# YuejiangDong/MAL

Hardware: AMD Instinct MI355X
Metric: train images/sec at B=12 192x640 KITTI-shaped (MAL loss path: passes A+B+C fwd+bwd) (higher is better)
Workload: dtype f32

## Files before the change

include/mal_hip.h:

```cpp
#ifndef MAL_HIP_H
#define MAL_HIP_H

#include <stddef.h>
#include <stdint.h>

#ifdef __cplusplus
extern "C" {
#endif

#define MAL_VERSION 100
#define MAL_MAX_FRAMES 2
#define MAL_MAX_CAND 4
#define MAL_MAX_INSTANCES 64
#define MAL_MATCH_MAX 128
#define MAL_INSTANCES_MAX_QK 16384
#define MAL_INSTANCES_MAX_K1 1025
#define MAL_INSTANCES_MAX_N 65535
#define MAL_MSDA_MAX_L 8
#define MAL_MSDA_MAX_P 8
#define MAL_MSDA_MAX_LP 32
#define MAL_MSDA_MAX_D 64

enum {
  MAL_OK = 0,
// ... 115 lines not shown

int mal_pose_fwd(const float* const* axisangle, const float* const* translation, const int* invert,
                 int B, int F, float* const* T, void* stream);
int mal_pose_bwd(const float* const* axisangle, const float* const* translation, const int* invert,
                 const float* const* g_T, int B, int F, float* const* g_axisangle ,
                 float* const* g_translation , void* stream);

enum {
  MAL_STEP_NO_ENS = 1,
  MAL_STEP_AUG_MASK = 2,
  MAL_STEP_TEMPORAL = 8,
  MAL_STEP_NOISE_PHILOX = 4,
  MAL_STEP_TEXEL_INPUTS = 64,
  MAL_STEP_DUAL_DISTIL = 32,
  MAL_STEP_SYN_SPARSE = 16,
  MAL_STEP_MAIN_TEMPORAL = 128,
  MAL_STEP_SYN_S_SPARSE = 256,
  MAL_STEP_NO_MOTION_MASK = 1024,
  MAL_STEP_NO_AUG = 2048,
  MAL_STEP_ENSEMBLE = 4096,
  MAL_STEP_NO_SSIM = 512
};
typedef struct mal_step_args {
  int B, H, W;
  float min_depth, max_depth;
  int flags;
  float w_main, w_distil;
  const float *color0, *color_m1, *color_p1;
  const float *K, *inv_K;
  const float *disp_teacher, *disp_student;
// ... 319 lines not shown
```

mal_amd/_lib.py:

```python
from __future__ import annotations

import ctypes as C
import os

import torch

_HERE = os.path.dirname(os.path.abspath(__file__))
LIB_PATH = os.environ.get("MAL_HIP_LIB") or os.path.join(_HERE, "lib", "libmal_hip.so")

c_fp = C.c_void_p
c_pp = C.c_void_p
i32, f32, sz, vp = C.c_int, C.c_float, C.c_size_t, C.c_void_p

SIGNATURES = {
    "mal_version": (i32, []),
    "mal_strerror": (C.c_char_p, [i32]),
    "mal_device_check": (i32, []),
    "mal_workspace_bytes": (sz, [i32, i32, i32]),
    "mal_disp_to_depth": (i32, [c_fp, sz, f32, f32, c_fp, c_fp, vp]),
    "mal_disp_to_depth_bwd": (i32, [c_fp, c_fp, c_fp, sz, f32, f32, c_fp, vp]),
    "mal_backproject": (i32, [c_fp, c_fp, i32, i32, i32, c_fp, vp]),
    "mal_backproject_bwd": (i32, [c_fp, c_fp, i32, i32, i32, c_fp, vp]),
    "mal_project3d": (i32, [c_fp, c_fp, c_fp, i32, i32, i32, f32, i32, c_fp, c_fp, vp]),
    "mal_project3d_bwd": (i32, [c_fp, c_fp, c_fp, c_fp, c_fp, i32, i32, i32, f32, i32, c_fp, c_fp, vp, sz, vp]),
# ... 185 lines not shown


class MsdaArgs(C.Structure):
    _fields_ = ([(n, vp) for n in ("value", "spatial_shapes", "level_start_index", "sampling_locations", "attention_weights",
                                   "reference_points")] +
                [(n, i32) for n in ("N", "S", "M", "D", "L", "P", "Lq", "ref_dim")] + [("out", vp), ("stream", vp)])


DR_MAX_ITERS = 4
MATCH_MAX,MATCH_U8, MATCH_F32 = 128, 0, 1
DR_NO_AUTOMASK, DR_NO_MOTION_MASK, DR_NOISE_PHILOX, DR_AVG, DR_NO_SSIM, DR_POSE_UPDATE = 1, 2, 4, 8, 16, 32
DR_POSE_NOISE_KEY = 0x706f73655f757064
MS_MAX_SCALES = 4
STEP_NO_ENS, STEP_AUG_MASK, STEP_NOISE_PHILOX, STEP_TEMPORAL, STEP_SYN_SPARSE, STEP_DUAL_DISTIL, STEP_TEXEL_INPUTS = 1, 2, 4, 8, 16, 32, 64
STEP_MAIN_TEMPORAL, STEP_SYN_S_SPARSE, STEP_NO_SSIM, STEP_NO_MOTION_MASK, STEP_NO_AUG, STEP_ENSEMBLE = 128, 256, 512, 1024, 2048, 4096
DEC_WIN, DEC_DISTIL, DEC_SMOOTH_X, DEC_SMOOTH_Y, DEC_TAP0, DEC_TAP1, DEC_L1, DEC_PLANES = 0, 1, 2, 3, 4, 5, 6, 7

F_AUTOMASK, F_GRAD, F_POSE_GRAD, F_NO_SSIM, F_AVG, F_EPILOGUE, F_DUAL_DISTIL, F_SRC_PACKED, F_TGT_PACKED = 1, 2, 4, 8, 16, 32, 64, 128, 256

_lib = None


class MalError(RuntimeError):
    pass


def load():
    global _lib
    if _lib is not None:
        return _lib
# ... 35 lines not shown
```

mal_amd/config.py:

```python
noise_source = "cpu"
noise_seed = 0x4d414c5eed
consistency_target = True
```

mal_amd/csrc/mal_march.h:

```cpp
#pragma once
#include "mal_common.h"
#include "mal_device.h"
#include "mal_pose.h"

namespace mal {

struct MarchParams {
  const float* disp; const float* disp2; const float* K; const float* invK;
  const float* T[2]; const float* src[2];
  const float* target; const float* ident; const float* noise; const float* ext_mask; const float* sample_scale;
  const float* mono_depth; const float* mono_reproj; const float* ens_reproj;
  const float* mono_disp; const float* lowest_cost; float* cmask_out;
  float merge_cons, merge_distil;
  const float* ens_disp; float* g_ens;
  int dual_distil;
  int avg, no_ssim;
  float* cam; int cam_ready;
  int sample_scale_is_mask;
  int B, H, W; float min_disp, range, eps; int convention;
  float* min_reproj; float* g_reproj; float* g_cons; float* g_distil; float* cons_target; float* depth_out;
  double* block_sums; float* block_gP;
  float* bnd;
  int strips, segs, rows, ntasks, per_xcd;
  int packed;
  int flip_odd;
  int debug;
  float* color_out[2]; unsigned char* argmin_out;
  float* min_reproj2; unsigned char* argmin_out2; float* weight_out;
  int color_out_stride;
  float* color_out2[2];
  const float* forced_w; const unsigned char* forced_arg; const float* g_color[2];
  const unsigned char* region;
  const float* fin_gn; const float* fin_coefs; const double* fin_stats; const float* fin_g_total; float* fin_out;
  unsigned* dbg;
  int framed; float* g_reproj2; float* bnd2;
};
constexpr int kDecPlanes = MAL_DEC_PLANES;

constexpr int kCamFloats = 40;

MAL_DEV void cam_fill(const float* K, const float* T0, const float* T1, const float* invK, float* cam, int b, int lane) {
  float mine = 0.f;
  if (lane < 24) {
    const int f = lane & 1, e = lane >> 1, i = e >> 2, j = e & 3;
    const float* Kb = K + b * 16;
    const float* T = (f ? T1 : T0) + b * 16;
    float acc = Kb[i * 4 + 0] * T[0 * 4 + j];
    acc = fma_(Kb[i * 4 + 1], T[1 * 4 + j], acc);
    acc = fma_(Kb[i * 4 + 2], T[2 * 4 + j], acc);
    mine = fma_(Kb[i * 4 + 3], T[3 * 4 + j], acc);
// ... 2 lines not shown
    mine = invK[b * 16 + (e / 3) * 4 + (e % 3)];
  }
  if (lane < kCamFloats) cam[b * kCamFloats + lane] = mine;
}

MarchParams march_params(int B, int H, int W, float min_depth, float max_depth, float eps, int convention);
int march_launch(MarchParams& p, int flags, hipStream_t st);
bool march_pair_qualifies(int B, int H, int W);
int march_pair_launch(MarchParams* ens, MarchParams& stu, int order, hipStream_t st);
void march_geometry(int B, int H, int W, int flags, int* strips, int* segs, int* rows);
inline int march_tasks_per_sample(int B, int H, int W, int flags) {
  int strips = 0, segs = 0;
  march_geometry(B, H, W, flags, &strips, &segs, nullptr);
  return strips * segs;
}
void step_geom_record(const void* ws, int B, int H, int W);
int step_geom_check(const void* ws, int B, int H, int W);
inline size_t march_bnd_floats(int B, int H, int W) { return (size_t)B * ((size_t)H / 8 + 1) * 2 * (size_t)W; }
MAL_DEV float march_boundary_term(const float* bnd, int b, int y, int x, int H, int W, int rows, int segs) {
  const int sq = y / rows, within = y - sq * rows;
  const int last = min(rows, H - sq * rows) - 1;
  float v = 0.f;
  if (within == 0 && sq > 0) v = bnd[((size_t)(b * segs + sq) * 2 + 0) * W + x];
  else if (within == last && sq < segs - 1) v = bnd[((size_t)(b * segs + sq) * 2 + 1) * W + x];
  return v;
}
MAL_DEV const float* march_boundary_row(const float* bnd, int b, int y, int H, int W, int rows, int segs) {
  const int sq = y / rows, within = y - sq * rows;
  const int last = min(rows, H - sq * rows) - 1;
  if (within == 0 && sq > 0) return bnd + ((size_t)(b * segs + sq) * 2 + 0) * W;
// ... 3 lines not shown
int pack_identity_tasks_per_sample(int H, int W);
struct StepPoses { PoseParams pose; const float* K; const float* invK; float* cam; unsigned* ticket; };
struct TieNoise { int on; unsigned long long seed, step; const unsigned long long* counter; float* noise_out ; };
struct SmoothParams { int n; const float* disp[2]; float* gn[2]; double* partials; unsigned* dec[2]; };
constexpr int kDrSlotsMax = 5;
struct DrExtra {
  const float* K; const float* invK; const float* T[kDrSlotsMax][2]; float* cam[kDrSlotsMax]; float* noise[kDrSlotsMax];
  unsigned long long seed, step; const unsigned long long* counter;
  int slots, pu_slot, noise_blocks, B, H, W; unsigned* ticket;
};
struct FusedMoreArgs {
  const float* target; const float* cand0; const float* cand1; int idx0; const float* ident; const float* noise;
  const float* prev_min; const uint8_t* prev_arg; float* min_reproj; uint8_t* argmin; float* weight_out; double* block_sums;
  float* g_cand0; float* g_cand1; const uint8_t* region; float* g_region0; float* g_region1; const float* orig0; const float* orig1;
  size_t orig_stride; int weight_given;
};
int photo_march_fused_more(const FusedMoreArgs& a, int B, int H, int W, int* per_sample_out, hipStream_t st,
                           unsigned* order = nullptr, unsigned* order_count = nullptr);
int photo_march_fused_more_n(int n, const FusedMoreArgs* a, int B, int H, int W, int* per_sample_out, hipStream_t st);
struct SmoothMapArgs { const float* disp; const float* img; int H, W; float* gn; double* partial; };
int smooth_march_sweep_batch(int n, const SmoothMapArgs* maps, int B, hipStream_t st, int* per_sample);
int smooth_march_batch_tasks(int H, int W);
hipStream_t side_begin(hipStream_t st);
int side_end(hipStream_t st);
int side_wait(hipStream_t st, bool always);
int tiebreak_noise_launch(unsigned long long seed, unsigned long long step, const unsigned long long* counter, unsigned mult,
                          int n, int B, int H, int W, float* const* out, hipStream_t st);
struct UpMaps { const float* src[2 * MAL_MS_MAX_SCALES]; float* dst[2 * MAL_MS_MAX_SCALES]; int h[2 * MAL_MS_MAX_SCALES], w[2 * MAL_MS_MAX_SCALES]; };
struct MsExtra {
  unsigned long long seed, step; const unsigned long long* counter; unsigned mult; int n_noise; float* noise[MAL_MS_MAX_SCALES];
  UpMaps up; int n_up;
// ... 154 lines not shown
```

mal_amd/csrc/mal_march.hip:

```cpp
#include "mal_march.h"
#include <atomic>
#include "mal_device.h"
#include "mal_pairs.h"
#include <mutex>
#include <unordered_map>

namespace mal {

#ifdef MAL_STAGE_MARKS
#define MAL_MARK(n) do { __builtin_amdgcn_sched_barrier(0); asm volatile("; MAL_STAGE " #n); __builtin_amdgcn_sched_barrier(0); } while (0)
#else
#define MAL_MARK(n) do { } while (0)
#endif

typedef __attribute__((address_space(4))) const float cfloat;

MAL_DEV void load_cam(const cfloat* cam, f2 (&P)[12], float (&ik)[9]) {
  asm volatile("" : "+s"(cam));
#pragma unroll
  for (int e = 0; e < 12; ++e) P[e] = (f2){cam[2 * e], cam[2 * e + 1]};
#pragma unroll
  for (int e = 0; e < 9; ++e) ik[e] = cam[24 + e];
}

// ... 373 lines not shown
  };
  auto maps_of = [&](CParams& pp) {
    Maps m;
    m.ident = AUTOMASK ? pp.ident : nullptr; m.noise = (AUTOMASK && !NO_NOISE) ? pp.noise : nullptr;
    m.ext_mask = EXT_NO ? nullptr : pp.ext_mask; m.lowest_cost = COST_NO ? nullptr : pp.lowest_cost;
    m.mono_disp = (COST_NO && !EPI) ? nullptr : pp.mono_disp;
    m.mono_depth = EPI ? pp.mono_depth : nullptr; m.mono_reproj = EPI ? pp.mono_reproj : nullptr;
    m.ens_reproj = EPI ? pp.ens_reproj : nullptr; m.target = pp.target; m.packed = LEAN ? 3 : pp.packed;
    m.forced_w = TEMPORAL ? pp.forced_w : nullptr; m.forced_arg = TEMPORAL ? pp.forced_arg : nullptr;
    m.gcol[0] = TEMPORAL ? pp.g_color[0] : nullptr; m.gcol[1] = TEMPORAL ? pp.g_color[1] : nullptr;
    m.fin_gn = TEMPORAL ? pp.fin_gn : nullptr;
    m.ens_disp = EPI ? pp.ens_disp : nullptr;
    return m;
  };
  auto row_of = [&](int rr) { return min(max(reflect1(rr, H), 0), H - 1); };
  auto request = [&](const Maps& pp, int rr, Ahead& a) {
    const bool packed_t = (pp.packed & 2) != 0;
    const unsigned pix = (unsigned)(prow(row_of(rr)) * W + gxr);
    const unsigned od = moff(row_of(rr));
    a.disp = ldf(disp_b, od);
    a.disp2 = 0.f;
    if (!NO_DISP2) {
      const float v = ldf(disp2_b ? disp2_b : disp_b, od);
      a.disp2 = disp2_b ? v : 0.f;
    }
    load_rgb(pp.target, packed_t, b, HW, pix, a.y);
    const unsigned oc = moff(min(max(rr - 1, 0), H - 1));
    auto opt = [&](const float* m, unsigned off, float absent) {
      const float v = ldf(m ? m : disp_b, off);
      return m ? v : absent;
    };
    a.ident = 0.f; a.noise = 0.f;
    if (AUTOMASK && !TEMPORAL) { a.ident = ldf(pp.ident, oc); if (!NO_NOISE) a.noise = opt(pp.noise, oc, 0.f); }
    if (TEMPORAL) {
      a.ident = ldf(pp.forced_w, oc);
      a.noise = (float)*(pp.forced_arg + (oc >> 2));
      const unsigned og = moff(min(max(rr - 2, 0), H - 1)) + 2u * (unsigned)b * (unsigned)HW * 4u;
#pragma unroll
      for (int ch = 0; ch < 3; ++ch) {
        const unsigned o = og + (unsigned)ch * (unsigned)HW * 4u;
#pragma unroll
        for (int f = 0; f < 2; ++f) a.gc[f * 3 + ch] = ldf(pp.gcol[f], o);
      }
    }
    a.ext = 1.f; a.mono = 0.f; a.cost = 1.f;
    if (EXT_YES) a.ext = ldf(pp.ext_mask, oc);
    else if (!EXT_NO) a.ext = opt(pp.ext_mask, oc, 1.f);
    if (COST_YES) {
      a.mono = ldf(pp.mono_disp, oc); a.cost = ldf(pp.lowest_cost, oc);
    } else if (!COST_NO) {
      a.mono = opt(pp.lowest_cost ? pp.mono_disp : nullptr, oc, 0.f);
      a.cost = opt(pp.lowest_cost, oc, 1.f);
    }
    const unsigned oq = GRAD ? moff(min(max(rr - 2, 0), H - 1)) : oc;
    a.e_mono = 0.f; a.e_mr = 0.f; a.e_er = 0.f; a.e_ensd = 0.f;
    if (EPI) {
      a.e_mono = ldf(MONO_YES ? pp.mono_disp : (pp.mono_disp ? pp.mono_disp : pp.mono_depth), oq);
// ... 969 lines not shown
}

int march_launch(MarchParams& p, int flags, hipStream_t st) {
  const bool grad = flags & MAL_F_GRAD, automask = flags & MAL_F_AUTOMASK, pose = flags & MAL_F_POSE_GRAD,
             epi = flags & MAL_F_EPILOGUE;
  march_decompose(p, flags);
  p.debug = g_debug;
  p.flip_odd = g_march_flip;
  p.packed = ((flags & MAL_F_SRC_PACKED) ? 1 : 0) | ((flags & MAL_F_TGT_PACKED) ? 2 : 0);
  dim3 grid(p.per_xcd * 8), block(64);
  if (!p.cam) return MAL_EINVAL;
  if ((long long)p.H * p.W >= (1ll << 24)) return MAL_ESHAPE;
  if (p.color_out[0] && (long long)p.B * (p.color_out_stride ? (long long)p.color_out_stride : 3ll * p.H * p.W) * 4 >= (1ll << 32))
    return MAL_ESHAPE;
  if (p.forced_w && (long long)p.B * 3 * p.H * p.W * 4 >= (1ll << 32)) return MAL_ESHAPE;
  if (!p.cam_ready) {
    hipLaunchKernelGGL(cam_setup_kernel, dim3(p.B), dim3(64), 0, st, p.K, p.T[0], p.T[1], p.invK, p.cam);
    p.cam_ready = 1;
  }
  const bool named = grad && pose && automask && !epi;
  hipEvent_t ev0 = named ? g_prof_start.exchange(nullptr) : nullptr, ev1 = named ? g_prof_stop.exchange(nullptr) : nullptr;
  if (ev0) (void)hipEventRecord(ev0, st);
  if ((p.avg || p.no_ssim) && (!grad || p.forced_w || p.color_out[0])) return MAL_EINVAL;
  const bool lean0 = g_march_lean && p.packed == 3 && !p.depth_out && p.debug == 0 && !p.dbg && !p.avg && !p.no_ssim &&
                     (long long)p.H * p.W * (kTexel * 4) < (1ll << 24);
  const bool no_maps = !p.ext_mask && !p.lowest_cost && !p.sample_scale;
  const bool conv_a = p.convention == 0, conv_b = p.convention == 1;
#ifdef MAL_CONV_FIXED
  const bool conv_teacher = conv_a;
#else
// ... 204 lines not shown
    if (m.h[k] < 1 || m.w[k] < 1 || m.h[k] > H || m.w[k] > W) return MAL_ESHAPE;
  }
  const MarchParams mp = march_params(B, H, W, min_depth, max_depth, 1e-7f, 0);
  WarpScalesParams p;
  p.m = m; p.src[0] = src[0]; p.src[1] = src[1]; p.cam = cam;
  p.B = B; p.H = H; p.W = W; p.stride = stride > 0 ? stride : 3 * H * W;
  p.min_disp = mp.min_disp; p.range = mp.range;
  const dim3 grid((W + 63) / 64, (H + 3) / 4, B * m.n), block(64, 4);
  if ((long long)H * W * (kTexel * 4) < (1ll << 24)) hipLaunchKernelGGL(warp_scales_kernel<true>, grid, block, 0, st, p);
  else hipLaunchKernelGGL(warp_scales_kernel<false>, grid, block, 0, st, p);
  return launch_status();
}

struct StepGeom {
  int rows_grad, rows_fwd, pack_rows, halo1;
  bool operator==(const StepGeom& o) const {
    return rows_grad == o.rows_grad && rows_fwd == o.rows_fwd && pack_rows == o.pack_rows && halo1 == o.halo1;
  }
};
static StepGeom step_geom_now(int B, int H, int W) {
  StepGeom g = {};
  march_geometry(B, H, W, MAL_F_GRAD, nullptr, nullptr, &g.rows_grad);
  march_geometry(B, H, W, 0, nullptr, nullptr, &g.rows_fwd);
  g.pack_rows = g_pack_rows;
  g.halo1 = g_march_halo1;
  return g;
}
static std::mutex g_geom_mutex;
static std::unordered_map<const void*, StepGeom> g_geom;

void step_geom_record(const void* ws, int B, int H, int W) {
  const StepGeom g = step_geom_now(B, H, W);
  std::lock_guard<std::mutex> lock(g_geom_mutex);
  if (g_geom.size() >= 4096 && !g_geom.count(ws)) g_geom.clear();
  g_geom[ws] = g;
}

int step_geom_check(const void* ws, int B, int H, int W) {
  const StepGeom g = step_geom_now(B, H, W);
  std::lock_guard<std::mutex> lock(g_geom_mutex);
// ... 166 lines not shown
```

mal_amd/csrc/mal_photo_march.hip:

```cpp
#include "mal_common.h"
#include "mal_device.h"
#include "mal_march.h"
#include "mal_pairs.h"

namespace mal {

struct PhotoMarchParams {
  const float* target; const float* cand[2];
  int target_texels;
  int weight_given;
  int idx[2];
  const float* ident; const float* noise; const float* ext_mask;
  const float* prev_min; const uint8_t* prev_arg;
  int last, automask;
  float* min_reproj; uint8_t* argmin; float* weight_out; double* block_sums;
  const uint8_t* argmin_in; const float* weight_in; const float* scale; const double* sums;
  float* g_cand[2];
  int B, H, W, strips, segs, rows, ntasks, per_xcd;
  const uint8_t* region;
  float* g_region[2];
  unsigned* order; unsigned* order_count;
  const float* orig[2]; size_t orig_stride;
};

struct Px9 { float t[3], a[3], c[3]; };

MAL_DEV void request9(const PhotoMarchParams& p, const float* tb, const float* ab, const float* cb, int HW, int row,
                      int gxr, Px9& q) {
  const unsigned bo = (unsigned)(row * p.W + gxr) * 4u;
  if (p.target_texels) {
    const texel_t t = ldt(tb, bo * (unsigned)kTexel);
    q.t[0] = t.x; q.t[1] = t.y; q.t[2] = t.z;
#pragma unroll
    for (int ch = 0; ch < 3; ++ch) { q.a[ch] = ldf(ab + (size_t)ch * HW, bo); q.c[ch] = ldf(cb + (size_t)ch * HW, bo); }
    return;
  }
#pragma unroll
// ... 140 lines not shown
  for (int i = 0; i < 9; ++i) { hsA[i] = bc(0.f); hsB[i] = bc(0.f); hcA[i] = bc(0.f); hcB[i] = bc(0.f); }
#pragma unroll
  for (int i = 0; i < 2; ++i) { hyA[i] = bc(0.f); hyB[i] = bc(0.f); hzA[i] = 0.f; hzB[i] = 0.f; }
  f2 x1[3] = {bc(0.f), bc(0.f), bc(0.f)}, x2[3] = {bc(0.f), bc(0.f), bc(0.f)}, y1rg = bc(0.f), y2rg = bc(0.f);
  float y1b = 0.f, y2b = 0.f;
  float w1 = 0.f;
  int win1 = 255;
  float acc_rw = 0.f, acc_w = 0.f;
  auto row_of = [&](int rr) { return min(max(reflect1(rr, H), 0), H - 1); };
  const uint8_t* rgn0 = (FUSED && p.region) ? p.region + map_b : nullptr;
  if (FUSED && rgn0) {
    unsigned any = 0u;
#pragma unroll 8
    for (int rr = max(y_lo - 2, 0); rr <= min(y_hi + 1, H - 1); ++rr) any |= rgn0[rr * W + gxr];
    if (!__any((any & 1u) && in_x)) {
      if (out_x)
        for (int c = y_lo; c < y_hi; ++c) {
          const unsigned o0 = (unsigned)(c * W + gxr) * 4u + img_b, o1 = o0 + hw4, o2 = o1 + hw4;
          stf(p.g_cand[0], o0, 0.f); stf(p.g_cand[0], o1, 0.f); stf(p.g_cand[0], o2, 0.f);
          if (p.g_cand[1]) { stf(p.g_cand[1], o0, 0.f); stf(p.g_cand[1], o1, 0.f); stf(p.g_cand[1], o2, 0.f); }
        }
      if (lane == 0) { p.block_sums[(size_t)task * 2] = 0.0; p.block_sums[(size_t)task * 2 + 1] = 0.0; }
      return;
    }
  }
  float nfA = 0.f, nfB = 0.f;
  const int r_first = max(y_lo - HALO, -1), r_last = y_hi - 1 + HALO;
  Px9 nxt;
  auto request9o = [&](CPhoto& P, int row, Px9& q) {
    const unsigned bo = (unsigned)(row * W + gxr) * 4u;
    const unsigned o0 = bo + img_b, o1 = o0 + hw4, o2 = o1 + hw4;
    if (FUSED) {
      const texel_t t = ldt(P.target, bo * (unsigned)kTexel + (unsigned)b * (unsigned)HW * (unsigned)(kTexel * 4));
      q.t[0] = t.x; q.t[1] = t.y; q.t[2] = t.z;
    } else {
      q.t[0] = ldf(P.target, o0); q.t[1] = ldf(P.target, o1); q.t[2] = ldf(P.target, o2);
    }
    q.a[0] = ldf(P.cand[0], o0); q.a[1] = ldf(P.cand[0], o1); q.a[2] = ldf(P.cand[0], o2);
    q.c[0] = ldf(P.cand[1], o0); q.c[1] = ldf(P.cand[1], o1); q.c[2] = ldf(P.cand[1], o2);
  };
// ... 423 lines not shown
    PhotoMarchParams p = {};
    p.target = target; p.B = B; p.H = H; p.W = W;
    const bool has2 = 2 * pr + 1 < n_cand;
    int i0 = 2 * pr, i1 = has2 ? 2 * pr + 1 : -1;
    if (!g_cand[i0] && i1 >= 0 && g_cand[i1]) { const int t = i0; i0 = i1; i1 = t; }
    if (!g_cand[i0]) continue;
    p.cand[0] = cand[i0]; p.idx[0] = i0; p.g_cand[0] = g_cand[i0];
    p.cand[1] = i1 >= 0 ? cand[i1] : cand[i0]; p.idx[1] = i1; p.g_cand[1] = i1 >= 0 ? g_cand[i1] : nullptr;
    p.argmin_in = argmin; p.weight_in = weight; p.scale = scale; p.sums = sums;
    decompose(p, 60, 2);
    hipLaunchKernelGGL(photo_march_bwd_kernel<false>, dim3(p.per_xcd * 8), dim3(64), 0, st, p);
  }
  return launch_status();
}

static int fused_more_params(PhotoMarchParams& p, const FusedMoreArgs& x, int B, int H, int W) {
  if (x.prev_min == x.min_reproj || x.prev_arg == x.argmin) return MAL_EINVAL;
  if (x.weight_given && x.noise) return MAL_EINVAL;
  if ((x.orig0 == nullptr) != (x.orig1 == nullptr) || (x.orig0 && !x.region)) return MAL_EINVAL;
  if ((long long)B * 3 * H * W * 4 >= (1ll << 32)) return MAL_ESHAPE;
  const size_t orig_stride = x.orig_stride ? x.orig_stride : (size_t)3 * H * W;
  if (x.orig0 && (long long)B * (long long)orig_stride * 4 >= (1ll << 32)) return MAL_ESHAPE;
  p = PhotoMarchParams{};
  p.target = x.target; p.target_texels = 1;
  p.weight_given = x.weight_given; p.B = B; p.H = H; p.W = W;
  p.cand[0] = x.cand0; p.cand[1] = x.cand1; p.idx[0] = x.idx0; p.idx[1] = x.idx0 + 1;
  p.prev_min = x.prev_min; p.prev_arg = x.prev_arg; p.ident = x.ident; p.noise = x.noise;
  p.min_reproj = x.min_reproj; p.argmin = x.argmin; p.weight_out = x.weight_out; p.block_sums = x.block_sums;
  p.g_cand[0] = x.g_cand0; p.g_cand[1] = x.g_cand1; p.region = x.region;
  p.orig[0] = x.orig0; p.orig[1] = x.orig1; p.orig_stride = orig_stride;
  if (x.region && x.g_region0 && x.g_region1) { p.g_region[0] = x.g_region0; p.g_region[1] = x.g_region1; }
  if (x.region && g_syn_rows >= 2 && g_syn_rows < 8) decompose(p, 60, 8, g_syn_rows);
  else decompose(p, 60, 2);
  return MAL_OK;
}
int photo_march_fused_more(const FusedMoreArgs& a, int B, int H, int W, int* per_sample_out, hipStream_t st, unsigned* order,
                           unsigned* order_count) {
  PhotoMarchParams p = {};
  int rc = fused_more_params(p, a, B, H, W);
  if (rc) return rc;
  *per_sample_out = p.strips * p.segs;
  unsigned grid = (unsigned)p.per_xcd * 8u;
#ifdef MAL_EXPERIMENTS
  if (a.region && order && order_count && g_syn_queue) {
    p.order = order; p.order_count = order_count;
    grid = (unsigned)p.ntasks;
    hipLaunchKernelGGL(photo_march_classify_kernel, dim3(grid), dim3(64), 0, st, p);
  }
#else
// ... 21 lines not shown
```

mal_amd/csrc/mal_step.hip:

```cpp
#include "mal_march.h"
#include "mal_device.h"
#include "mal_pose.h"
#include "mal_pairs.h"
#include "mal_tail.h"
#include <mutex>

namespace mal {

constexpr int kLossSlots = 16;
constexpr int kEpiBlocks = 64;

opt_t g_march_halo1{1};
opt_t g_step_overlap{1};
opt_t g_temporal_spec{0};
opt_t g_side_priority{0};
opt_t g_student_overlap{2};
opt_t g_side_order{0};
opt_t g_tail_overlap{1};
opt_t g_sweeps_batched{1};

struct StepWs {
  float* packed[3];
  float* T[2]; float* gT[2]; float* gTs[2];
  float* ident; float* mono_reproj; float* ens_reproj;
  float* G_r_t; float* G_r_s; float* G_c; float* gn_t; float* gn_s;
  float* G_e;
  float* multi_reproj;
  double* bs_d;
  double* bs_t; double* bs_s; double* bs_e; float* bgP;
  float* bgP_e;
  double* bs_p;
  unsigned char* arg_t; float* w_t; double* bs_ph;
  float* rp_warp; unsigned char* arg_warp;
  unsigned char* arg_s; float* w_s; double* bs_sh; float* rp_warp_s; unsigned char* arg_warp_s;
  double* ps;
  unsigned* ticket;
  unsigned* order;
  double* sm_stats;
  float* coefs;
  float* cam;
  float* bnd_t; float* bnd_s;
  size_t bytes;
};

static StepWs carve_step(void* base, int B, int H, int W) {
  StepWs w;
  char* p = (char*)base;
// ... 16 lines not shown
  w.rp_warp = (float*)take(map);
  w.arg_warp = (unsigned char*)take((size_t)B * HW);
  w.arg_s = (unsigned char*)take((size_t)B * HW);
  w.w_s = (float*)take(map);
  w.bs_sh = (double*)take(nb * 4 * 2 * 8);
  w.rp_warp_s = (float*)take(map);
  w.arg_warp_s = (unsigned char*)take((size_t)B * HW);
  w.ps = (double*)take((size_t)2 * B * 8 * 8);
  w.ticket = (unsigned*)take(16);
  w.order = (unsigned*)take(nb * 4 * sizeof(unsigned));
  w.sm_stats = (double*)take((size_t)4 * B * 8);
  w.coefs = (float*)take(16 * 4);
  w.cam = (float*)take((size_t)B * 40 * 4);
  w.bnd_t = (float*)take(march_bnd_floats(B, H, W) * 4);
  w.bnd_s = (float*)take(march_bnd_floats(B, H, W) * 4);
  w.bytes = o;
  return w;
}

struct EpiParams {
  const float *disp_s, *disp_t, *mono_reproj, *ens_reproj, *multi_reproj, *ext_mask, *lowest_cost, *sample_scale, *ens_disp;
  int scale_is_mask, dual;
  int skip_dead;
  float min_disp, range, merge_cons, merge_distil;
  float *G_c, *G_e; double* partials; unsigned* dbg; int B, HW;
};
MAL_DEV void step_epilogue_block(const EpiParams& p, int bid) {
  __shared__ double s_red[2][4];
  const int b = bid / kEpiBlocks, blk = bid - b * kEpiBlocks, tid = threadIdx.x;
  const int per = (p.HW + kEpiBlocks - 1) / kEpiBlocks, lo = blk * per, hi = min(lo + per, p.HW);
// ... 643 lines not shown
      m.out[k][0] = student ? sc->warp_s_m1[s] : sc->warp_m1[s];
      m.out[k][1] = student ? sc->warp_s_p1[s] : sc->warp_p1[s];
      m.out2[k][0] = student ? sc->warp2_s_m1[s] : sc->warp2_m1[s];
      m.out2[k][1] = student ? sc->warp2_s_p1[s] : sc->warp2_p1[s];
      if (!m.disp[k] || !m.out[k][0] || !m.out[k][1] || (m.out2[k][0] == nullptr) != (m.out2[k][1] == nullptr)) return MAL_EINVAL;
    }
  }
  rc = step_check(a);
  if (rc) return rc;
  const StepWs w = step_ws(a);
  const float* src[2] = {w.packed[1], w.packed[2]};
  return warp_scales_launch(m, src, w.cam, a->B, a->H, a->W, a->min_depth, a->max_depth, a->warp_sample_stride,
                            (hipStream_t)a->stream);
}

static FusedMoreArgs teacher_sweep(const mal_step_args* a, const StepWs& w, float* mono_reproj) {
  const bool sparse = (a->flags & MAL_STEP_SYN_SPARSE) != 0;
  FusedMoreArgs x = {};
  x.target = w.packed[0]; x.cand0 = a->syn_m1; x.cand1 = a->syn_p1; x.idx0 = 2; x.ident = w.ident; x.noise = a->noise;
  x.prev_min = w.rp_warp; x.prev_arg = w.arg_warp; x.min_reproj = mono_reproj; x.argmin = w.arg_t; x.weight_out = w.w_t;
  x.block_sums = w.bs_ph; x.g_cand0 = a->g_syn_m1; x.g_cand1 = a->g_syn_p1; x.region = a->syn_region;
  x.g_region0 = a->g_syn_region_m1; x.g_region1 = a->g_syn_region_p1;
  x.orig0 = sparse ? a->warp_m1 : nullptr; x.orig1 = sparse ? a->warp_p1 : nullptr; x.orig_stride = (size_t)a->warp_sample_stride;
  return x;
}
static FusedMoreArgs student_sweep(const mal_step_args* a, const StepWs& w) {
  const bool sparse = (a->flags & MAL_STEP_SYN_S_SPARSE) != 0;
  FusedMoreArgs x = {};
  x.target = w.packed[0]; x.cand0 = a->syn_s_m1; x.cand1 = a->syn_s_p1; x.idx0 = 2;
  x.ident = w.w_s; x.weight_given = 1;
  x.prev_min = w.rp_warp_s; x.prev_arg = w.arg_warp_s; x.min_reproj = a->multi_reproj ? a->multi_reproj : w.multi_reproj;
  x.argmin = w.arg_s; x.weight_out = w.w_s; x.block_sums = w.bs_sh; x.g_cand0 = a->g_syn_s_m1; x.g_cand1 = a->g_syn_s_p1;
  x.region = a->syn_s_region; x.g_region0 = a->g_syn_s_region_m1; x.g_region1 = a->g_syn_s_region_p1;
  x.orig0 = sparse ? a->warp_s_m1 : nullptr; x.orig1 = sparse ? a->warp_s_p1 : nullptr; x.orig_stride = (size_t)a->warp_sample_stride;
  return x;
}
static int sweep_check(const FusedMoreArgs& x, bool sparse) {
  if (!x.cand0 || !x.cand1 || !x.g_cand0 || !x.g_cand1) return MAL_EINVAL;
// ... 120 lines not shown
  float* mono_reproj = a->mono_reproj ? a->mono_reproj : w.mono_reproj;
  for (int i = 0; i < launches; ++i) {
    rc = launch_teacher(a, w, mono_reproj, (hipStream_t)a->stream);
    if (rc) return rc;
  }
  return MAL_OK;
}

static int launch_teacher_temporal(const mal_step_args* a, const StepWs& w, SideStream* tail, hipStream_t st, int* per_sample_t,
                                   bool* teacher_done) {
  if (!a->g_warp_m1 || !a->g_warp_p1) return MAL_EINVAL;
  MarchParams p = teacher_params(a, w, nullptr);
  p.g_reproj = w.G_r_t; p.block_sums = w.bs_t;
  p.ident = w.ident;
  p.forced_w = w.w_t; p.forced_arg = w.arg_t; p.g_color[0] = a->g_warp_m1; p.g_color[1] = a->g_warp_p1;
  if (g_temporal_spec) {
    p.region = a->syn_region; p.block_sums = w.bs_e;
  } else if (tail) {
    p.block_sums = w.bs_e;
  } else {
    p.fin_gn = w.gn_t; p.fin_coefs = w.coefs; p.fin_stats = w.sm_stats; p.fin_g_total = a->g_total; p.fin_out = a->g_disp_teacher;
    *teacher_done = a->g_disp_teacher != nullptr;
  }
  p.bnd = halo_bnd(w.bnd_t);
  p.dbg = a->dec_teacher;
  const int rc = march_launch(p, MAL_F_AUTOMASK | MAL_F_GRAD | MAL_F_POSE_GRAD | MAL_F_SRC_PACKED | MAL_F_TGT_PACKED, st);
  *per_sample_t = p.strips * p.segs;
  return rc;
}
static int step_bwd_body(const mal_step_args* a, const StepWs& w, SideStream* tail, hipStream_t st) {
// ... 48 lines not shown
```

mal_amd/step.py:

```python
from __future__ import annotations

import contextlib
import ctypes as C
import inspect
from collections import namedtuple
from typing import Any, NamedTuple

import torch
from torch.autograd import Function
from torch.autograd.function import once_differentiable

from . import _lib as L
from . import config, loss_utils, ops

_NOISE_COUNTER = {}


class StepConsts(NamedTuple):
    color0: Any; color_m1: Any; color_p1: Any; K: Any; inv_K: Any
    cmask: Any; keep: Any
    lowest: Any; noise: Any


class StepCfg(NamedTuple):
    min_depth: float; max_depth: float; no_ens: bool; w_main: float; w_distil: float; want_maps: bool; aug_is_mask: bool
    want_decisions: bool
    philox: Any
    dual_distil: bool = False

# ... 211 lines not shown
        sc = self.scale or 0
        out[("color", -1, sc)], out[("color", 1, sc)] = self.warp
        if syn is not None and region is None:
            out[("syn", -1, sc)], out[("syn", 1, sc)] = syn
        elif syn is not None and dense:
            inside = (region & 1).bool().unsqueeze(1)
            out[("syn", -1, sc)], out[("syn", 1, sc)] = (torch.where(inside, t, w_) for t, w_ in zip(syn, self.warp))


class _Hint(_HintIO):

    def __init__(self, a, student, B, H, W, dev, scale=None):
        new = lambda shape: torch.empty(shape, dtype=torch.float32, device=dev)
        super().__init__(a, student, scale, new((B, 2, 3, H, W)), [new((B, 3, H, W)) for _ in range(2)])
        self.sparse_flag = L.STEP_SYN_S_SPARSE if student else L.STEP_SYN_SPARSE
        self.sparse = False
        self.shape, self.dev = (B, 3, H, W), dev
        self.region, self.snap, self.syn, self.syn_data, self.leaf, self.g_syn = None, None, None, None, None, None

    def _mark_sparse(self):
        self.sparse = True
        if self.scale is None:
            self.a.flags |= self.sparse_flag
        else:
            self.a.syn_sparse |= 1 << self.scale

    def produce(self, synth, inputs, defer=False):
        with torch.enable_grad():
            self.leaf = [w.detach().requires_grad_(True) for w in self.warp]
            self._call(synth, inputs, self.leaf)
        if not defer:
# ... 17 lines not shown
                                           and region.is_contiguous()):
                raise L.MalError("loss_step: ('syn_region', %d) must be a contiguous (B,H,W) uint8 device tensor" % sc)
            self.region = region
            if region is not None:
                self._put("syn" + self.tag + "_region", region.data_ptr())
                if sparse:
                    self._mark_sparse()
                self.snap = [torch.empty(self.shape, dtype=torch.float32, device=self.dev) for _ in range(2)]
                self._set("g_syn", self.snap, ("_region_m1", "_region_p1"))
        else:
            self.syn, self.syn_data = None, self.pre
            self.region = torch.zeros((B, H, W), dtype=torch.uint8, device=self.dev)
            self._put("syn" + self.tag + "_region", self.region.data_ptr())
            self._mark_sparse()
        self.g_syn = [torch.empty(self.shape, dtype=torch.float32, device=self.dev) for _ in range(2)]
        self._set("syn", self.syn_data)
        self._set("g_syn", self.g_syn)

    def expose(self, out, dense):
        self._expose(out, dense, self.syn_data if self.has_ins else None, self.region if self.sparse else None)
        out["multi_has_ins" if self.student else "has_ins"] = self.has_ins

    def backward(self, stream=None):
        on_stream = False
        if self.syn is None:
            g_warp = self.g_syn
            on_stream = stream is not None
        else:
            from . import dyn_utils
            reg = {g.data_ptr(): (self.snap[i] if self.snap is not None else None) for i, g in enumerate(self.g_syn)}
            dyn_utils.INPLACE_COTANGENTS.update(reg)
            dyn_utils.BACKWARD_STREAM["handle"], dyn_utils.BACKWARD_STREAM["used"] = stream, False
            try:
                g_warp = torch.autograd.grad(self.syn, self.leaf, self.g_syn, allow_unused=True)
            finally:
                for k in reg:
                    dyn_utils.INPLACE_COTANGENTS.pop(k, None)
                used = dyn_utils.BACKWARD_STREAM["used"]
                dyn_utils.BACKWARD_STREAM["handle"], dyn_utils.BACKWARD_STREAM["used"] = None, False
            on_stream = bool(used) and all(g is not None and g.data_ptr() == q.data_ptr() and g.is_contiguous()
                                           for g, q in zip(g_warp, self.g_syn))
            g_warp = [torch.zeros_like(w) if g is None else g.contiguous() for g, w in zip(g_warp, self.warp)]
        self.g_warp = g_warp
        self._set("g_warp", g_warp)
        return on_stream


def _scale_buffers(dev, B, H, W, student, s):
    new = lambda shape: torch.empty(shape, dtype=torch.float32, device=dev)
    return _cached("scale_hint", dev, (B, H, W, student, s), lambda: (new((B, 2, 3, H, W)), new((B, 3, H, W)), new((B, 3, H, W))))


class _ScaleHint(_HintIO):

    def __init__(self, sa, student, s, B, H, W, dev):
        pair, pre0, pre1 = _scale_buffers(dev, B, H, W, student, s)
# ... 365 lines not shown
```

Before: 41520.

## Keep synthesised-pair cotangent sparse by skipping dense zero-fill of dead tiles

The teacher photo-march sweep no longer zero-fills the gradient buffers of tiles with no region pixels. Instead it records a per-tile liveness byte, and the temporal march kernel consults that map through a wavefront ballot to skip loading color gradients from dead rows, substituting zeros. This removes dense zero-store and load traffic on the cotangent buffers when the synthesis region is sparse. In exchange it adds validation, a geometry coupling between the two kernels, a Python-side check that the producer's backward runs in place, and a debug NaN-poison option.

```diff
diff --git a/include/mal_hip.h b/include/mal_hip.h
--- a/include/mal_hip.h
+++ b/include/mal_hip.h
@@ -153,6 +153,7 @@
   MAL_STEP_TEXEL_INPUTS = 64,
   MAL_STEP_DUAL_DISTIL = 32,
   MAL_STEP_SYN_SPARSE = 16,
+  MAL_STEP_GSYN_SPARSE = 8192,
   MAL_STEP_MAIN_TEMPORAL = 128,
   MAL_STEP_SYN_S_SPARSE = 256,
   MAL_STEP_NO_MOTION_MASK = 1024,
diff --git a/mal_amd/_lib.py b/mal_amd/_lib.py
--- a/mal_amd/_lib.py
+++ b/mal_amd/_lib.py
@@ -223,6 +223,7 @@
 MS_MAX_SCALES = 4
 STEP_NO_ENS, STEP_AUG_MASK, STEP_NOISE_PHILOX, STEP_TEMPORAL, STEP_SYN_SPARSE, STEP_DUAL_DISTIL, STEP_TEXEL_INPUTS = 1, 2, 4, 8, 16, 32, 64
 STEP_MAIN_TEMPORAL, STEP_SYN_S_SPARSE, STEP_NO_SSIM, STEP_NO_MOTION_MASK, STEP_NO_AUG, STEP_ENSEMBLE = 128, 256, 512, 1024, 2048, 4096
+STEP_GSYN_SPARSE = 8192
 DEC_WIN, DEC_DISTIL, DEC_SMOOTH_X, DEC_SMOOTH_Y, DEC_TAP0, DEC_TAP1, DEC_L1, DEC_PLANES = 0, 1, 2, 3, 4, 5, 6, 7
 
 F_AUTOMASK, F_GRAD, F_POSE_GRAD, F_NO_SSIM, F_AVG, F_EPILOGUE, F_DUAL_DISTIL, F_SRC_PACKED, F_TGT_PACKED = 1, 2, 4, 8, 16, 32, 64, 128, 256
diff --git a/mal_amd/config.py b/mal_amd/config.py
--- a/mal_amd/config.py
+++ b/mal_amd/config.py
@@ -1,3 +1,6 @@
+import os
+
 noise_source = "cpu"
 noise_seed = 0x4d414c5eed
 consistency_target = True
+syn_grad_sparse = os.environ.get("MAL_SYN_GRAD_SPARSE", "1") != "0"
diff --git a/mal_amd/csrc/mal_march.h b/mal_amd/csrc/mal_march.h
--- a/mal_amd/csrc/mal_march.h
+++ b/mal_amd/csrc/mal_march.h
@@ -34,6 +34,7 @@
   const float* fin_gn; const float* fin_coefs; const double* fin_stats; const float* fin_g_total; float* fin_out;
   unsigned* dbg;
   int framed; float* g_reproj2; float* bnd2;
+  const unsigned char* g_color_live; int live_rows, live_strips, live_segs;
 };
 constexpr int kDecPlanes = MAL_DEC_PLANES;
 
@@ -66,6 +67,7 @@
   march_geometry(B, H, W, flags, &strips, &segs, nullptr);
   return strips * segs;
 }
+inline bool march_live_rows_fit(int rows) { return rows + 2 <= 64; }
 void step_geom_record(const void* ws, int B, int H, int W);
 int step_geom_check(const void* ws, int B, int H, int W);
 inline size_t march_bnd_floats(int B, int H, int W) { return (size_t)B * ((size_t)H / 8 + 1) * 2 * (size_t)W; }
@@ -99,7 +101,9 @@
   const float* prev_min; const uint8_t* prev_arg; float* min_reproj; uint8_t* argmin; float* weight_out; double* block_sums;
   float* g_cand0; float* g_cand1; const uint8_t* region; float* g_region0; float* g_region1; const float* orig0; const float* orig1;
   size_t orig_stride; int weight_given;
-};
+  uint8_t* tile_live;
+};
+void photo_march_fused_geometry(int B, int H, int W, bool region, int* strips, int* segs, int* rows);
 int photo_march_fused_more(const FusedMoreArgs& a, int B, int H, int W, int* per_sample_out, hipStream_t st,
                            unsigned* order = nullptr, unsigned* order_count = nullptr);
 int photo_march_fused_more_n(int n, const FusedMoreArgs* a, int B, int H, int W, int* per_sample_out, hipStream_t st);
diff --git a/mal_amd/csrc/mal_march.hip b/mal_amd/csrc/mal_march.hip
--- a/mal_amd/csrc/mal_march.hip
+++ b/mal_amd/csrc/mal_march.hip
@@ -411,6 +411,11 @@
     return m;
   };
   auto row_of = [&](int rr) { return min(max(reflect1(rr, H), 0), H - 1); };
+  unsigned long long live_rows = ~0ull;
+  if (TEMPORAL && p.g_color_live) {
+    const int yy = min(max(ph_lo - 1 + lane, 0), H - 1);
+    live_rows = __ballot(p.g_color_live[(b * p.live_segs + yy / p.live_rows) * p.live_strips + strip] != 0);
+  }
   auto request = [&](const Maps& pp, int rr, Ahead& a) {
     const bool packed_t = (pp.packed & 2) != 0;
     const unsigned pix = (unsigned)(prow(row_of(rr)) * W + gxr);
@@ -432,12 +437,18 @@
     if (TEMPORAL) {
       a.ident = ldf(pp.forced_w, oc);
       a.noise = (float)*(pp.forced_arg + (oc >> 2));
-      const unsigned og = moff(min(max(rr - 2, 0), H - 1)) + 2u * (unsigned)b * (unsigned)HW * 4u;
-#pragma unroll
-      for (int ch = 0; ch < 3; ++ch) {
-        const unsigned o = og + (unsigned)ch * (unsigned)HW * 4u;
-#pragma unroll
-        for (int f = 0; f < 2; ++f) a.gc[f * 3 + ch] = ldf(pp.gcol[f], o);
+      const int gq = min(max(rr - 2, 0), H - 1);
+      const unsigned og = moff(gq) + 2u * (unsigned)b * (unsigned)HW * 4u;
+      if ((live_rows >> ((prow(gq) - (ph_lo - 1)) & 63)) & 1ull) {
+#pragma unroll
+        for (int ch = 0; ch < 3; ++ch) {
+          const unsigned o = og + (unsigned)ch * (unsigned)HW * 4u;
+#pragma unroll
+          for (int f = 0; f < 2; ++f) a.gc[f * 3 + ch] = ldf(pp.gcol[f], o);
+        }
+      } else {
+#pragma unroll
+        for (int i = 0; i < 6; ++i) a.gc[i] = 0.f;
       }
     }
     a.ext = 1.f; a.mono = 0.f; a.cost = 1.f;
@@ -1437,6 +1448,9 @@
   if (p.color_out[0] && (long long)p.B * (p.color_out_stride ? (long long)p.color_out_stride : 3ll * p.H * p.W) * 4 >= (1ll << 32))
     return MAL_ESHAPE;
   if (p.forced_w && (long long)p.B * 3 * p.H * p.W * 4 >= (1ll << 32)) return MAL_ESHAPE;
+  if (p.g_color_live && (!p.forced_w || !grad || p.live_rows < 1 || p.live_strips != p.strips ||
+                         p.live_segs != (p.H + p.live_rows - 1) / p.live_rows || !march_live_rows_fit(p.rows)))
+    return MAL_EINVAL;
   if (!p.cam_ready) {
     hipLaunchKernelGGL(cam_setup_kernel, dim3(p.B), dim3(64), 0, st, p.K, p.T[0], p.T[1], p.invK, p.cam);
     p.cam_ready = 1;
@@ -1671,8 +1685,10 @@
 
 struct StepGeom {
   int rows_grad, rows_fwd, pack_rows, halo1;
+  int syn_rows;
   bool operator==(const StepGeom& o) const {
-    return rows_grad == o.rows_grad && rows_fwd == o.rows_fwd && pack_rows == o.pack_rows && halo1 == o.halo1;
+    return rows_grad == o.rows_grad && rows_fwd == o.rows_fwd && pack_rows == o.pack_rows && halo1 == o.halo1 &&
+           syn_rows == o.syn_rows;
   }
 };
 static StepGeom step_geom_now(int B, int H, int W) {
@@ -1681,6 +1697,7 @@
   march_geometry(B, H, W, 0, nullptr, nullptr, &g.rows_fwd);
   g.pack_rows = g_pack_rows;
   g.halo1 = g_march_halo1;
+  g.syn_rows = g_syn_rows;
   return g;
 }
 static std::mutex g_geom_mutex;
diff --git a/mal_amd/csrc/mal_photo_march.hip b/mal_amd/csrc/mal_photo_march.hip
--- a/mal_amd/csrc/mal_photo_march.hip
+++ b/mal_amd/csrc/mal_photo_march.hip
@@ -21,6 +21,7 @@
   float* g_region[2];
   unsigned* order; unsigned* order_count;
   const float* orig[2]; size_t orig_stride;
+  uint8_t* tile_live;
 };
 
 struct Px9 { float t[3], a[3], c[3]; };
@@ -191,7 +192,9 @@
 #pragma unroll 8
     for (int rr = max(y_lo - 2, 0); rr <= min(y_hi + 1, H - 1); ++rr) any |= rgn0[rr * W + gxr];
     if (!__any((any & 1u) && in_x)) {
-      if (out_x)
+      if (p.tile_live) {
+        if (lane == 0) p.tile_live[task] = 0;
+      } else if (out_x)
         for (int c = y_lo; c < y_hi; ++c) {
           const unsigned o0 = (unsigned)(c * W + gxr) * 4u + img_b, o1 = o0 + hw4, o2 = o1 + hw4;
           stf(p.g_cand[0], o0, 0.f); stf(p.g_cand[0], o1, 0.f); stf(p.g_cand[0], o2, 0.f);
@@ -201,6 +204,7 @@
       return;
     }
   }
+  if (FUSED && p.tile_live && lane == 0) p.tile_live[task] = 1;
   float nfA = 0.f, nfB = 0.f;
   const int r_first = max(y_lo - HALO, -1), r_last = y_hi - 1 + HALO;
   Px9 nxt;
@@ -654,6 +658,10 @@
   return launch_status();
 }
 
+static void fused_decompose(PhotoMarchParams& p, bool region) {
+  if (region && g_syn_rows >= 2 && g_syn_rows < 8) decompose(p, 60, 8, g_syn_rows);
+  else decompose(p, 60, 2);
+}
 static int fused_more_params(PhotoMarchParams& p, const FusedMoreArgs& x, int B, int H, int W) {
   if (x.prev_min == x.min_reproj || x.prev_arg == x.argmin) return MAL_EINVAL;
   if (x.weight_given && x.noise) return MAL_EINVAL;
@@ -670,9 +678,18 @@
   p.g_cand[0] = x.g_cand0; p.g_cand[1] = x.g_cand1; p.region = x.region;
   p.orig[0] = x.orig0; p.orig[1] = x.orig1; p.orig_stride = orig_stride;
   if (x.region && x.g_region0 && x.g_region1) { p.g_region[0] = x.g_region0; p.g_region[1] = x.g_region1; }
-  if (x.region && g_syn_rows >= 2 && g_syn_rows < 8) decompose(p, 60, 8, g_syn_rows);
-  else decompose(p, 60, 2);
+  if (x.tile_live && !x.region) return MAL_EINVAL;
+  p.tile_live = x.tile_live;
+  fused_decompose(p, x.region != nullptr);
   return MAL_OK;
+}
+void photo_march_fused_geometry(int B, int H, int W, bool region, int* strips, int* segs, int* rows) {
+  PhotoMarchParams p = {};
+  p.B = B; p.H = H; p.W = W;
+  fused_decompose(p, region);
+  if (strips) *strips = p.strips;
+  if (segs) *segs = p.segs;
+  if (rows) *rows = p.rows;
 }
 int photo_march_fused_more(const FusedMoreArgs& a, int B, int H, int W, int* per_sample_out, hipStream_t st, unsigned* order,
                            unsigned* order_count) {
diff --git a/mal_amd/csrc/mal_step.hip b/mal_amd/csrc/mal_step.hip
--- a/mal_amd/csrc/mal_step.hip
+++ b/mal_amd/csrc/mal_step.hip
@@ -31,6 +31,7 @@
   float* bgP_e;
   double* bs_p;
   unsigned char* arg_t; float* w_t; double* bs_ph;
+  unsigned char* tile_live;
   float* rp_warp; unsigned char* arg_warp;
   unsigned char* arg_s; float* w_s; double* bs_sh; float* rp_warp_s; unsigned char* arg_warp_s;
   double* ps;
@@ -77,6 +78,7 @@
   w.cam = (float*)take((size_t)B * 40 * 4);
   w.bnd_t = (float*)take(march_bnd_floats(B, H, W) * 4);
   w.bnd_s = (float*)take(march_bnd_floats(B, H, W) * 4);
+  w.tile_live = (unsigned char*)take(nb * 4);
   w.bytes = o;
   return w;
 }
@@ -750,6 +752,13 @@
                             (hipStream_t)a->stream);
 }
 
+static bool gsyn_sparse(const mal_step_args* a) {
+  const int need = MAL_STEP_TEMPORAL | MAL_STEP_SYN_SPARSE | MAL_STEP_GSYN_SPARSE;
+  if ((a->flags & need) != need || !a->syn_region || g_temporal_spec) return false;
+  int rows = 0;
+  march_geometry(a->B, a->H, a->W, MAL_F_GRAD, nullptr, nullptr, &rows);
+  return march_live_rows_fit(rows);
+}
 static FusedMoreArgs teacher_sweep(const mal_step_args* a, const StepWs& w, float* mono_reproj) {
   const bool sparse = (a->flags & MAL_STEP_SYN_SPARSE) != 0;
   FusedMoreArgs x = {};
@@ -758,6 +767,7 @@
   x.block_sums = w.bs_ph; x.g_cand0 = a->g_syn_m1; x.g_cand1 = a->g_syn_p1; x.region = a->syn_region;
   x.g_region0 = a->g_syn_region_m1; x.g_region1 = a->g_syn_region_p1;
   x.orig0 = sparse ? a->warp_m1 : nullptr; x.orig1 = sparse ? a->warp_p1 : nullptr; x.orig_stride = (size_t)a->warp_sample_stride;
+  x.tile_live = gsyn_sparse(a) ? w.tile_live : nullptr;
   return x;
 }
 static FusedMoreArgs student_sweep(const mal_step_args* a, const StepWs& w) {
@@ -908,6 +918,11 @@
   p.g_reproj = w.G_r_t; p.block_sums = w.bs_t;
   p.ident = w.ident;
   p.forced_w = w.w_t; p.forced_arg = w.arg_t; p.g_color[0] = a->g_warp_m1; p.g_color[1] = a->g_warp_p1;
+  if (gsyn_sparse(a)) {
+    if (a->g_warp_m1 != a->g_syn_m1 || a->g_warp_p1 != a->g_syn_p1) return MAL_EINVAL;
+    p.g_color_live = w.tile_live;
+    photo_march_fused_geometry(a->B, a->H, a->W, true, &p.live_strips, &p.live_segs, &p.live_rows);
+  }
   if (g_temporal_spec) {
     p.region = a->syn_region; p.block_sums = w.bs_e;
   } else if (tail) {
diff --git a/mal_amd/step.py b/mal_amd/step.py
--- a/mal_amd/step.py
+++ b/mal_amd/step.py
@@ -13,6 +13,7 @@
 from . import _lib as L
 from . import config, loss_utils, ops
 
+POISON_COTANGENTS = False
 _NOISE_COUNTER = {}
 
 
@@ -254,7 +255,7 @@
         new = lambda shape: torch.empty(shape, dtype=torch.float32, device=dev)
         super().__init__(a, student, scale, new((B, 2, 3, H, W)), [new((B, 3, H, W)) for _ in range(2)])
         self.sparse_flag = L.STEP_SYN_S_SPARSE if student else L.STEP_SYN_SPARSE
-        self.sparse = False
+        self.sparse, self.gsyn_sparse = False, False
         self.shape, self.dev = (B, 3, H, W), dev
         self.region, self.snap, self.syn, self.syn_data, self.leaf, self.g_syn = None, None, None, None, None, None
 
@@ -302,8 +303,30 @@
             self._put("syn" + self.tag + "_region", self.region.data_ptr())
             self._mark_sparse()
         self.g_syn = [torch.empty(self.shape, dtype=torch.float32, device=self.dev) for _ in range(2)]
+        if POISON_COTANGENTS:
+            for g in self.g_syn:
+                g.fill_(float("nan"))
         self._set("syn", self.syn_data)
         self._set("g_syn", self.g_syn)
+        self.gsyn_sparse = self._cotangent_never_read_densely()
+        if self.gsyn_sparse:
+            self.a.flags |= L.STEP_GSYN_SPARSE
+
+    def _cotangent_never_read_densely(self):
+        if not config.syn_grad_sparse or self.student or self.scale is not None or not self.sparse:
+            return False
+        if self.syn is None:
+            return True
+        return self.snap is not None and self._producer_on_leaves()
+
+    def _producer_on_leaves(self):
+        from . import dyn_utils
+        fn = self.syn[0].grad_fn
+        if fn is None or fn is not self.syn[1].grad_fn or not isinstance(fn, dyn_utils.BatchSynthesisFn._backward_cls):
+            return False
+        nxt = fn.next_functions
+        return len(nxt) >= 2 and all(nxt[i][0] is not None and getattr(nxt[i][0], "variable", None) is self.leaf[i]
+                                     for i in range(2))
 
     def expose(self, out, dense):
         self._expose(out, dense, self.syn_data if self.has_ins else None, self.region if self.sparse else None)
@@ -318,7 +341,8 @@
             from . import dyn_utils
             reg = {g.data_ptr(): (self.snap[i] if self.snap is not None else None) for i, g in enumerate(self.g_syn)}
             dyn_utils.INPLACE_COTANGENTS.update(reg)
-            dyn_utils.BACKWARD_STREAM["handle"], dyn_utils.BACKWARD_STREAM["used"] = stream, False
+            dyn_utils.BACKWARD_STREAM["handle"] = stream if self._producer_on_leaves() else None
+            dyn_utils.BACKWARD_STREAM["used"] = False
             try:
                 g_warp = torch.autograd.grad(self.syn, self.leaf, self.g_syn, allow_unused=True)
             finally:
@@ -326,8 +350,11 @@
                     dyn_utils.INPLACE_COTANGENTS.pop(k, None)
                 used = dyn_utils.BACKWARD_STREAM["used"]
                 dyn_utils.BACKWARD_STREAM["handle"], dyn_utils.BACKWARD_STREAM["used"] = None, False
-            on_stream = bool(used) and all(g is not None and g.data_ptr() == q.data_ptr() and g.is_contiguous()
-                                           for g, q in zip(g_warp, self.g_syn))
+            in_place = all(g is not None and g.data_ptr() == q.data_ptr() and g.is_contiguous() for g, q in zip(g_warp, self.g_syn))
+            if self.gsyn_sparse and not in_place:
+                raise L.MalError("loss_step backward: the producer's backward did not take its in-place, region-only form, but "
+                                 "the step kept the cotangent of the synthesised pair sparse (config.syn_grad_sparse)")
+            on_stream = bool(used) and in_place
             g_warp = [torch.zeros_like(w) if g is None else g.contiguous() for g, w in zip(g_warp, self.warp)]
         self.g_warp = g_warp
         self._set("g_warp", g_warp)
```

After: 42300, median of 6. 1.02x the previous value.
